# modal-labs/modal-client

Hardware: AMD Instinct MI355X
Metric: map_items_per_sec (higher is better)
Workload: dtype bf16; 1 GPU; model=Function.map fan-out (BASELINE config 3), global_batch=12500, seq_len=0, parallelism=map1, dynamic_batching=64, chunk_items=256, workers=8

## Files before the change

### csrc/core.cpp

```cpp

#include <pybind11/pybind11.h>
#include <pybind11/stl.h>

#include "lane.h"
#include "ring.h"

#include <algorithm>
#include <atomic>
#include <functional>
#include <thread>
#include <cerrno>
#include <cstdint>
#include <cstring>
#include <fcntl.h>
#include <stdexcept>
#include <string>
#include <sys/mman.h>
#include <sys/stat.h>
#include <unistd.h>
#include <vector>

namespace py = pybind11;

namespace {

using modal_amd::BellFile;
using modal_amd::Ring;
using modal_amd::RingHub;

constexpr uint64_t kGilReleaseBytes = 64 * 1024;

bool ring_push(Ring& ring, py::buffer buf) {
  py::buffer_info info = buf.request();
  const uint8_t* src = static_cast<const uint8_t*>(info.ptr);
  const uint64_t n = (uint64_t)info.size * (uint64_t)info.itemsize;
  uint8_t* dst = ring.reserve(n);
  if (!dst) return false;
  if (n >= kGilReleaseBytes) {
    py::gil_scoped_release release;
    std::memcpy(dst, src, n);
  } else {
    std::memcpy(dst, src, n);
  }
  ring.commit();
  return true;
}

py::list ring_pop_all(Ring& ring, size_t max_frames) {
  py::list out;
  ring.pop(
      [&](const uint8_t* ptr, size_t len) {
        out.append(py::bytes(reinterpret_cast<const char*>(ptr), len));
      },
      max_frames);
  return out;
}

py::list hub_drain(RingHub& hub) {
  py::list out;
  hub.drain([&](int slot, const uint8_t* ptr, size_t len) {
    out.append(py::make_tuple(slot, py::bytes(reinterpret_cast<const char*>(ptr), len)));
  });
  return out;
}

using modal_amd::Assignment;
using modal_amd::ChunkDone;
using modal_amd::ChunkLane;
using modal_amd::FrameKind;

py::str sv_str(std::string_view s) { return py::str(s.data(), s.size()); }

py::tuple done_tuple(const ChunkDone& d) {
  py::object cis = py::none();
  if (!d.cis_nil) {
    py::list items;
    for (int64_t v : d.cis) items.append(py::int_(v));
    cis = std::move(items);
// ... 367 lines not shown
    ::close(cg_fd);
    cg_fd = -1;
    throw std::runtime_error("clone3(CLONE_INTO_CGROUP) unavailable: " +
                             std::string(strerror(errno)));
  }
  if (pid < 0) {
    if (cg_fd >= 0) ::close(cg_fd);
    throw std::runtime_error("clone3: " + std::string(strerror(errno)));
  }
  if (pid == 0) {
    ::setsid();
    if (stdin_fd >= 0) ::dup2(stdin_fd, 0);
    if (stdout_fd >= 0) ::dup2(stdout_fd, 1);
    if (stderr_fd >= 0) ::dup2(stderr_fd, 2);
    for (int fd = 3; fd < 1024; ++fd) ::close(fd);
    if (!cwd.empty() && ::chdir(cwd.c_str()) != 0) _exit(126);
    if (rlimit_as_mib > 0) {
      struct rlimit rl;
      rl.rlim_cur = rl.rlim_max = (rlim_t)rlimit_as_mib << 20;
      ::setrlimit(RLIMIT_AS, &rl);
    }
    ::execve(cargv[0], cargv.data(), cenv.data());
    _exit(127);
  }
  if (cg_fd >= 0) ::close(cg_fd);
  return (int64_t)pid;
}


PYBIND11_MODULE(_core, m) {
  m.doc() = "modal_amd native core: shm ring transport + batch framing";
  py::class_<BellFile, std::shared_ptr<BellFile>>(m, "BellFile")
      .def(py::init<const std::string&, bool>(), py::arg("path"), py::arg("create") = false);
  py::class_<Ring, std::shared_ptr<Ring>>(m, "ShmRing")
      .def(py::init<const std::string&, uint64_t, bool>(), py::arg("path"),
           py::arg("capacity") = (uint64_t)64 << 20, py::arg("create") = false)
      .def("push", &ring_push)
      .def("pop_all", &ring_pop_all, py::arg("max_frames") = 0)
      .def("pending_bytes", &Ring::pending_bytes)
      .def("capacity", &Ring::capacity)
      .def("too_large", &Ring::too_large)
      .def("bell_wakes", &Ring::bell_wakes)
      .def("set_shared_bell", &Ring::set_shared_bell);
  py::class_<RingHub>(m, "RingHub")
      .def(py::init<const std::string&, int>(), py::arg("bell_path") = "",
           py::arg("timeout_ms") = 20)
      .def("add_ring", &RingHub::add_ring)
      .def("remove_ring", &RingHub::remove_ring)
      .def("fd", &RingHub::fd)
      .def("drain", &hub_drain)
      .def("close", &RingHub::close)
      .def("stats", [](RingHub& hub) {
        py::dict d;
        d["notifies"] = hub.notifies();
        d["waits"] = hub.waits();
        d["drains"] = hub.drains();
        d["producer_wakes"] = hub.producer_wakes();
        d["rings"] = hub.ring_count();
        return d;
      });
  py::class_<ChunkLane>(m, "ChunkLane")
      .def(py::init<>())
      .def("add_worker", &ChunkLane::add_worker)
      .def("remove_worker", &ChunkLane::remove_worker)
      .def("set_eligible", &ChunkLane::set_eligible)
      .def("set_cap", &ChunkLane::set_cap, py::arg("fn_slot"), py::arg("items"),
           py::arg("min_chunks") = 1)
// ... 30 lines not shown
```

### csrc/lane_stress.cpp

```cpp

#include <poll.h>

#include <atomic>
#include <cstdio>
#include <cstdlib>
#include <map>
#include <string>
#include <thread>
#include <vector>

#include "lane.h"
#include "ring.h"

using namespace modal_amd;

namespace {

constexpr int kWorkers = 2;
constexpr int kChunks = 20000;
constexpr uint64_t kRingBytes = 64 * 1024;
constexpr uint64_t kCount = 64;
constexpr uint64_t kCapItems = 128;
constexpr uint32_t kMinChunks = 2;

#define CHECK(cond)                                                      \
  do {                                                                   \
    if (!(cond)) {                                                       \
      std::fprintf(stderr, "CHECK failed: %s (line %d)\n", #cond, __LINE__); \
      std::abort();                                                      \
    }                                                                    \
  } while (0)

void put_str(std::string& out, const std::string& s) {
  if (s.size() < 32) {
    out.push_back((char)(0xa0 | s.size()));
  } else {
    out.push_back((char)0xd9);
    out.push_back((char)s.size());
  }
  out += s;
}

std::string encode_done(const std::string& token, uint64_t count, const std::string& data) {
  std::string out;
  out.push_back((char)0x88);
  put_str(out, "t");
  put_str(out, "chunk_done");
  put_str(out, "token");
  put_str(out, token);
  put_str(out, "call_id");
  put_str(out, "fc-stress");
  put_str(out, "chunk_id");
  put_str(out, token.substr(2));
  put_str(out, "function_id");
  put_str(out, "fu-stress");
  put_str(out, "count");
  out.push_back((char)count);
  put_str(out, "data");
  out.push_back((char)0xc5);
  out.push_back((char)(data.size() >> 8));
  out.push_back((char)(data.size() & 0xff));
  out += data;
  put_str(out, "cis");
  out.push_back((char)0xc0);
  return out;
}

std::string make_frame(int seq) {
  std::string head = std::to_string(seq) + ":";
  size_t len = 1024 + (size_t)((seq * 2654435761u) % 3072);
  std::string out = head;
  out.resize(len, (char)('a' + seq % 26));
  return out;
}

bool wait_fd(int fd, int timeout_ms) {
  struct pollfd pfd = {fd, POLLIN, 0};
  return ::poll(&pfd, 1, timeout_ms) > 0;
}

}

int main() {
  char dir_template[] = "/tmp/lane-stress-XXXXXX";
  CHECK(::mkdtemp(dir_template) != nullptr);
  std::string dir = dir_template;

  std::vector<std::shared_ptr<Ring>> to_worker_tx, to_worker_rx, from_worker_tx, from_worker_rx;
  for (int i = 0; i < kWorkers; i++) {
    std::string in = dir + "/in." + std::to_string(i), outp = dir + "/out." + std::to_string(i);
    to_worker_tx.push_back(std::make_shared<Ring>(in, kRingBytes, true));
    to_worker_rx.push_back(std::make_shared<Ring>(in, 0, false));
    from_worker_tx.push_back(std::make_shared<Ring>(outp, kRingBytes, true));
    from_worker_rx.push_back(std::make_shared<Ring>(outp, 0, false));
  }

  std::atomic<bool> stop{false};
  std::atomic<int> answered{0};

  std::thread worker([&] {
    RingHub hub(dir + "/worker.bell", 20);
    for (int i = 0; i < kWorkers; i++) hub.add_ring(i, to_worker_rx[i]);
    auto sched_bell = std::make_shared<BellFile>(dir + "/sched.bell", true);
    for (int i = 0; i < kWorkers; i++) from_worker_tx[i]->set_shared_bell(sched_bell);
    std::vector<int> last_seq(kWorkers, -1);
    std::vector<std::pair<int, std::string>> replies;
    while (!stop.load()) {
      wait_fd(hub.fd(), 50);
      replies.clear();
      hub.drain([&](int slot, const uint8_t* ptr, size_t len) {
        std::string body(reinterpret_cast<const char*>(ptr), len);
        int seq = std::atoi(body.c_str());
        CHECK(body == make_frame(seq));
// ... 42 lines not shown
        submitted++;
        if (slot >= 0) assigned(token, slot);
      }
      wait_fd(hub.fd(), 50);
      assignments.clear();
      std::vector<std::pair<int, std::string>> done_now;
      lane.drain(
          hub,
          [&](int slot, const ChunkDone& done) {
            CHECK(done.count == (int64_t)kCount && done.cis_nil);
            CHECK(done.data.size() == (size_t)(std::atoi(done.token.data() + 2) % 700));
            done_now.emplace_back(slot, std::string(done.token));
          },
          [&](int, const uint8_t*, size_t) { CHECK(false && "no raw frames expected"); },
          &assignments);
      for (auto& d : done_now) {
        auto it = where.find(d.second);
        CHECK(it != where.end() && it->second == d.first);
        where.erase(it);
        held[d.first] -= kCount;
        completed++;
      }
      for (auto& a : assignments) assigned(a.token, a.worker_slot);
    }
    CHECK(where.empty() && lane.queued(0) == 0);
    CHECK(lane.pushed() == (uint64_t)kChunks);
    std::printf("lane_stress ok: %d chunks, hub notifies=%llu waits=%llu producer_wakes=%llu\n",
                completed, (unsigned long long)hub.notifies(), (unsigned long long)hub.waits(),
                (unsigned long long)hub.producer_wakes());
    stop.store(true);
    worker.join();
  }
  CHECK(answered.load() == kChunks);
  std::string cmd = "rm -rf " + dir;
  return std::system(cmd.c_str()) == 0 ? 0 : 1;
}
```

### csrc/ring.h

```cpp

#pragma once

#include <atomic>
#include <cerrno>
#include <climits>
#include <cstdint>
#include <cstring>
#include <ctime>
#include <fcntl.h>
#include <linux/futex.h>
#include <memory>
#include <csignal>
#include <pthread.h>
#include <mutex>
#include <stdexcept>
#include <string>
#include <sys/eventfd.h>
#include <sys/mman.h>
#include <sys/stat.h>
#include <sys/syscall.h>
#include <thread>
#include <unistd.h>
#include <utility>
#include <vector>
// ... 92 lines not shown
      ::close(fd_);
      throw std::runtime_error("ShmRing: mmap failed");
    }
    base_ = static_cast<uint8_t*>(mem);
    header_ = reinterpret_cast<RingHeader*>(base_);
    data_ = base_ + sizeof(RingHeader);
    total_ = total;
    if (create) {
      header_->head.store(0, std::memory_order_relaxed);
      header_->tail.store(0, std::memory_order_relaxed);
      header_->capacity = capacity;
      header_->bell.seq.store(0, std::memory_order_relaxed);
      header_->bell.waiting.store(0, std::memory_order_relaxed);
      header_->bell.wakes.store(0, std::memory_order_relaxed);
      header_->magic = kMagic;
    } else if (header_->magic != kMagic || header_->capacity != capacity) {
      ::munmap(base_, total_);
      ::close(fd_);
      throw std::runtime_error("ShmRing: magic mismatch");
    }
    capacity_ = capacity;
  }

  ~Ring() {
    if (base_) ::munmap(base_, total_);
    if (fd_ >= 0) ::close(fd_);
  }

  Ring(const Ring&) = delete;
  Ring& operator=(const Ring&) = delete;

  bool too_large(uint64_t n) const { return n + 8 > capacity_ || n >= kSkip; }

  uint8_t* reserve(uint64_t n) {
    if (too_large(n)) throw std::runtime_error("frame larger than ring");
    uint64_t head = header_->head.load(std::memory_order_relaxed);
    uint64_t tail = header_->tail.load(std::memory_order_acquire);
    uint64_t pos = head % capacity_;
    uint64_t to_end = capacity_ - pos;
    uint64_t need = 4 + n;
    uint64_t skip = to_end < need ? to_end : 0;
    if (head + skip + need - tail > capacity_) return nullptr;
    if (skip) {
      if (to_end >= 4) {
        uint32_t sentinel = kSkip;
        std::memcpy(data_ + pos, &sentinel, 4);
      }
      pos = 0;
    }
    uint32_t len32 = (uint32_t)n;
    std::memcpy(data_ + pos, &len32, 4);
    pending_commit_ = head + skip + need;
    return data_ + pos + 4;
  }

  void commit() {
    header_->head.store(pending_commit_, std::memory_order_release);
    bell_ring(header_->bell);
    if (shared_bell_) bell_ring(*shared_bell_->bell());
  }

  bool push(const uint8_t* src, uint64_t n) {
    uint8_t* dst = reserve(n);
    if (!dst) return false;
    std::memcpy(dst, src, n);
    commit();
    return true;
  }

  template <typename F>
  size_t pop(F&& cb, size_t max_frames = 0) {
    uint64_t tail = header_->tail.load(std::memory_order_relaxed);
    uint64_t head = header_->head.load(std::memory_order_acquire);
    if (tail == head) return 0;
    size_t count = 0;
    while (tail < head) {
      uint64_t pos = tail % capacity_;
      uint64_t to_end = capacity_ - pos;
      if (to_end < 4) {
        tail += to_end;
        continue;
      }
      uint32_t len32;
      std::memcpy(&len32, data_ + pos, 4);
      if (len32 == kSkip) {
        tail += to_end;
        continue;
      }
      if ((uint64_t)len32 + 4 > to_end || tail + 4 + len32 > head) break;
      cb(static_cast<const uint8_t*>(data_ + pos + 4), (size_t)len32);
      tail += 4 + len32;
      if (max_frames && ++count >= max_frames) break;
    }
    header_->tail.store(tail, std::memory_order_release);
    return count;
  }

  bool has_pending() const {
    return header_->head.load(std::memory_order_acquire) !=
           header_->tail.load(std::memory_order_acquire);
  }

  uint64_t pending_bytes() const {
    return header_->head.load(std::memory_order_acquire) -
           header_->tail.load(std::memory_order_acquire);
  }

  uint64_t capacity() const { return capacity_; }
  Bell* bell() const { return &header_->bell; }
  uint32_t bell_wakes() const { return header_->bell.wakes.load(std::memory_order_relaxed); }

  void set_shared_bell(std::shared_ptr<BellFile> bell) { shared_bell_ = std::move(bell); }

 private:
  int fd_ = -1;
  uint8_t* base_ = nullptr;
  uint8_t* data_ = nullptr;
  RingHeader* header_ = nullptr;
  uint64_t capacity_ = 0;
  uint64_t total_ = 0;
  uint64_t pending_commit_ = 0;
  std::shared_ptr<BellFile> shared_bell_;
};

class RingHub {
 public:
  explicit RingHub(const std::string& bell_path = "", int timeout_ms = 20)
      : timeout_ms_(timeout_ms < 1 ? 1 : timeout_ms) {
    if (!bell_path.empty()) {
      bell_file_ = std::make_shared<BellFile>(bell_path, true);
      bell_ = bell_file_->bell();
    }
    efd_ = ::eventfd(0, EFD_NONBLOCK | EFD_CLOEXEC);
    if (efd_ < 0) throw std::runtime_error("RingHub: eventfd failed");
    thread_ = std::thread([this] { run(); });
  }

  ~RingHub() { close(); }
  RingHub(const RingHub&) = delete;
  RingHub& operator=(const RingHub&) = delete;

  void add_ring(int slot, std::shared_ptr<Ring> ring) {
    std::lock_guard<std::mutex> lock(mu_);
    for (auto& entry : rings_) {
      if (entry.first == slot) {
        entry.second = std::move(ring);
        return;
      }
    }
    if (!bell_) {
      bell_owner_ = ring;
      bell_ = ring->bell();
    }
    rings_.emplace_back(slot, std::move(ring));
  }
// ... 118 lines not shown
```

### modal_amd/runtime/worker.py

```python

from __future__ import annotations

import asyncio
import contextvars
import inspect
import os
import sys
import time
import traceback
from concurrent.futures import ThreadPoolExecutor
from typing import Any, Optional

from .._serialization import (
    DataFormat,
    GeneratorDone,
    deserialize,
    deserialize_payload,
    serialize,
    serialize_data_format,
    set_client_context,
)
from ..scheduler.blobs import INLINE_LIMIT, BlobStore
from ..scheduler.calls import (
    GENERIC_STATUS_FAILURE,
# ... 23 lines not shown
    try:
        return (
            cuda is not None
            and os.environ.get("MODAL_AMD_SLOT_STREAMS", "0") not in ("0", "false")
            and cuda.is_initialized()
        )
    except AttributeError:
        return False


def _invoke_on_slot_stream(fn: Any, args: tuple, kwargs: dict) -> Any:
    torch = sys.modules.get("torch")
    cuda = getattr(torch, "cuda", None) if torch is not None else None
    try:
        if (
            cuda is None
            or os.environ.get("MODAL_AMD_SLOT_STREAMS", "0") in ("0", "false")
            or not cuda.is_initialized()
        ):
            return fn(*args, **kwargs)
    except AttributeError:
        return fn(*args, **kwargs)
    stream = getattr(_slot_tls, "stream", None)
    if stream is None:
        stream = torch.cuda.Stream()
        _slot_tls.stream = stream
    with torch.cuda.stream(stream):
        result = fn(*args, **kwargs)
    ev = torch.cuda.Event()
    ev.record(stream)
    torch.cuda.default_stream().wait_event(ev)
    return result

RUNTIME: Optional["WorkerRuntime"] = None


class WorkerRPCTarget:

    def __init__(self, runtime: "WorkerRuntime"):
        self._runtime = runtime

    async def tensor_pull(self, token: str) -> Optional[bytes]:
        tensor = self._runtime.tensor_table.get(token)
        if tensor is None:
            return None
        import pickle as _pickle

        loop = asyncio.get_running_loop()
        return await loop.run_in_executor(
            None, lambda: _pickle.dumps(tensor.detach().cpu(), 4)
        )

    async def ping(self) -> str:
        return self._runtime.task_id

    async def app_stop(self, app_id: str) -> bool:
        await self._runtime._app_teardown(app_id)
        return True

    async def gpu_snapshot(self) -> dict:
        rt = self._runtime
        async with rt.snapshot_lock:
            if rt.mem_snapshot is not None:
                return {"state": rt.mem_snapshot.state.value}
            from .gpu_snapshot import GPUMemorySnapshot

            snap = GPUMemorySnapshot()
            await asyncio.get_running_loop().run_in_executor(None, snap.checkpoint)
            rt.mem_snapshot = snap
            return {"state": snap.state.value}

    async def exec_command(self, cmd: list, timeout: float = 60.0) -> dict:
        proc = await asyncio.create_subprocess_exec(
            *cmd,
            stdout=asyncio.subprocess.PIPE,
            stderr=asyncio.subprocess.STDOUT,
            env=dict(os.environ),
        )
        try:
            out, _ = await asyncio.wait_for(proc.communicate(), timeout)
        except asyncio.TimeoutError:
            proc.kill()
            return {"returncode": -1, "output": "(timed out)"}
        return {"returncode": proc.returncode, "output": out[-65536:].decode(errors="replace")}

    async def gpu_restore(self) -> dict:
        rt = self._runtime
# ... 15 lines not shown
        if float_codec not in (False, True, "auto"):
            raise InvalidError(f'float_codec is False, True or "auto", got {float_codec!r}')
        return await asyncio.get_running_loop().run_in_executor(
            None, capture_manifest, self._runtime.blob_store, float_codec
        )


class FunctionRuntime:

    def __init__(self, runtime: "WorkerRuntime", msg: dict):
        self.runtime = runtime
        self.function_id = msg["function_id"]
        self.app_id = msg.get("app_id", "")
        self.name = msg.get("name", "")
        self.is_generator = bool(msg.get("is_generator"))
        self.timeout = msg.get("timeout")
        self.max_concurrent = max(int(msg.get("max_concurrent_inputs") or 1), 1)
        self.batch_max_size = int(msg.get("batch_max_size") or 0)
        self.batch_linger_ms = int(msg.get("batch_linger_ms") or 0)
        self.version = msg.get("version", 1)
        self.definition_blob = msg["definition"]
        self.definition_kind = msg.get("definition_kind", "serialized")
        self.env = msg.get("env") or {}
        self.volumes = msg.get("volumes") or {}
        self.python_paths = msg.get("python_paths") or []
        self.web_config = msg.get("web_config")
        self._web_runtime: Any = None
        self.sem = asyncio.Semaphore(self.max_concurrent)
        self._callable: Any = None
        self._service: Any = None
        self._loaded = False
        self._load_error: Optional[BaseException] = None
        self._enter_done = False
        self._batch: list[tuple[dict, tuple, dict]] = []
        self._batch_flush_handle: Optional[asyncio.TimerHandle] = None

    def load(self) -> Any:
        if self._loaded:
            if self._load_error is not None:
                raise self._load_error
            return self._callable
        try:
            if self.env:
                os.environ.update(self.env)
            for p in self.python_paths:
                if p not in sys.path:
                    sys.path.insert(0, p)
            if self.volumes:
                from .volumes import mount_volumes

                mount_volumes(self.volumes, self.runtime)
            obj = deserialize(self.definition_blob)
            if isinstance(obj, dict) and obj.get("kind") == "cls_service":
                self._service = _ClsService(obj)
                self._callable = None
            else:
                self._callable = obj
            self._loaded = True
            return self._callable
        except BaseException as exc:
            self._load_error = exc
            self._loaded = True
            raise

    def get_callable(self, method_name: str) -> Any:
        fn = self.load()
# ... 88 lines not shown
        self.gpu_index = (
            int(os.environ["MODAL_AMD_GPU_INDEX"]) if "MODAL_AMD_GPU_INDEX" in os.environ else None
        )
        self.socket_path = os.environ["MODAL_AMD_WORKER_SOCKET"]
        self.external = os.environ.get("MODAL_AMD_EXTERNAL_WORKER") == "1"
        self.conn: Optional[Connection] = None
        self.task_id: str = ""
        self.functions: dict[str, FunctionRuntime] = {}
        self.mem_snapshot: Any = None
        self.snapshot_lock = asyncio.Lock()
        self._sync_threads: dict[str, set] = {}
        self._sync_threads_lock = _threading.Lock()
        self.executor = ThreadPoolExecutor(
            max_workers=int(os.environ.get("MODAL_AMD_WORKER_THREADS", "16")),
            thread_name_prefix="modal-amd-input",
        )
        run_dir = os.path.dirname(self.socket_path)
        self.blob_store = BlobStore(os.path.join(run_dir, "blobs"))
        from .devicemesh import DeviceMesh, TensorTable

        self.mesh = DeviceMesh()
        self.tensor_table = TensorTable()
        self._chunk_cache: dict[str, dict] = {}
        self._chunk_order: list[str] = []
        self._outbox: list[dict] = []
        self._outbox_flush_scheduled = False
        self._running: dict[str, asyncio.Task] = {}
        self._abandoned: set[str] = set()
        self._shutdown = asyncio.Event()
        self._hello_ack = asyncio.Event()
        self._log_buffer: list[tuple[int, str]] = []
        self._log_flush_scheduled = False
        self.loop: Optional[asyncio.AbstractEventLoop] = None

    async def run(self) -> None:
        global RUNTIME
        RUNTIME = self
        self.loop = asyncio.get_running_loop()
        if os.environ.get("MODAL_AMD_RESTORE_STATE_PATH"):
            from .gpu_snapshot import wait_and_restore_from_state_file

            await asyncio.get_running_loop().run_in_executor(
                None, wait_and_restore_from_state_file
            )
        deadline = time.time() + (60.0 if self.external else 0.0)
        while True:
            try:
                reader, writer = await asyncio.open_unix_connection(self.socket_path)
                break
            except (FileNotFoundError, ConnectionRefusedError):
                if time.time() >= deadline:
                    return
                await asyncio.sleep(0.05)
        self.conn = Connection(reader, writer, self._handle, rpc_target=WorkerRPCTarget(self))
        self.conn.start()
        from ..scheduler.core import read_auth_token

        await self.conn.send(
            {
                "t": "hello",
                "role": "worker",
                "worker_id": self.worker_id,
                "gpu_index": self.gpu_index,
                "external": self.external,
                "pid": os.getpid(),
                "auth": read_auth_token(self.socket_path),
# ... 34 lines not shown
            return None
        try:
            free, total = torch.cuda.mem_get_info()
            return {
                "hbm_total": total,
                "hbm_free": free,
                "hbm_reserved": torch.cuda.memory_reserved(),
            }
        except Exception:
            return None

    async def _heartbeat_loop(self) -> None:
        while True:
            await asyncio.sleep(HEARTBEAT_INTERVAL)
            try:
                msg: dict = {"t": "hb"}
                stats = self._gpu_stats()
                if stats:
                    msg["gpu"] = stats
                await self.conn.send(msg)
            except Exception:
                return

    def _handle_sync(self, msg: dict) -> bool:
        if msg.get("t") != "inputs_chunk":
            return False
        frt = self.functions.get(msg["function_id"])
        if frt is None:
            return False
        self._start_chunk(frt, msg)
        return True

    def _start_chunk(self, frt: "FunctionRuntime", msg: dict) -> None:
        task = asyncio.get_running_loop().create_task(self._run_chunk(frt, msg))
        self._running[msg["token"]] = task
        task.add_done_callback(lambda _t, tok=msg["token"]: self._running.pop(tok, None))

    async def _handle(self, msg: dict) -> None:
        kind = msg.get("t")
        if kind == "hello_ack":
            self.task_id = msg.get("task_id", "")
            os.environ["MODAL_AMD_TASK_ID"] = self.task_id
            if msg.get("ring_in"):
                attached = self.conn.attach_rings(
                    msg.get("ring_out"), msg.get("ring_in"), create=False
                )
                if attached and msg.get("lane_bell"):
                    self.conn.sync_handler = self._handle_sync
                    attached = self.conn.enable_lane(shared_bell=msg["lane_bell"], own_hub=True)
                if msg.get("lane_bell") and not attached:
                    sys.__stderr__.write(
                        f"worker {self.worker_id}: cannot attach the native lane, closing\n"
                    )
                    self._shutdown.set()
                    return
            self._hello_ack.set()
        elif kind == "def":
            frt = FunctionRuntime(self, msg)
            self.functions[frt.function_id] = frt
        elif kind == "inputs":
            for cid, data in (msg.get("chunks") or {}).items():
                self._chunk_cache[cid] = {"raw": data, "decoded": None}
                self._chunk_order.append(cid)
                while len(self._chunk_order) > 512:
                    old = self._chunk_order.pop(0)
                    self._chunk_cache.pop(old, None)
            frt = self.functions.get(msg["function_id"])
# ... 255 lines not shown
                vid, ro, _sub = mount_spec(spec)
                if not ro:
                    volume_ids.add(vid)
            if frt._service is not None:
                await asyncio.get_running_loop().run_in_executor(
                    self.executor, frt._service.exit
                )
        if volume_ids:
            await asyncio.get_running_loop().run_in_executor(None, os.sync)
            for volume_id in volume_ids:
                try:
                    await self.conn.call("volume_commit", {"volume_id": volume_id}, timeout=10)
                except Exception:
                    pass

    def _setup_cluster(self, cluster: dict) -> None:
        from ..experimental import ClusterInfo, _set_cluster_info

        rank, size = cluster["rank"], cluster["size"]
        os.environ["RANK"] = str(rank)
        os.environ["WORLD_SIZE"] = str(size)
        os.environ["LOCAL_RANK"] = "0"
        os.environ["MASTER_ADDR"] = "127.0.0.1"
        os.environ["MASTER_PORT"] = str(cluster["master_port"])
        _set_cluster_info(
            ClusterInfo(
                rank=rank,
                cluster_id=cluster["cluster_id"],
                container_ips=["127.0.0.1"] * size,
                fabric_ids=[0] * size,
            )
        )

    async def _run_chunk(self, frt: FunctionRuntime, msg: dict) -> None:
        count = msg["count"]
        token = msg["token"]
        call_id = msg["call_id"]
        self._chunk_cache[msg["chunk_id"]] = {"raw": msg.get("payload"), "decoded": None}
        self._chunk_order.append(msg["chunk_id"])
        while len(self._chunk_order) > 512:
            old = self._chunk_order.pop(0)
            self._chunk_cache.pop(old, None)
        loop = asyncio.get_running_loop()

        values: dict[int, Any] = {}
        errors: dict[int, tuple] = {}

        def run_range(start: int, end: int) -> None:
            try:
                fn = frt.get_callable(msg.get("method", ""))
                pairs, kw_common = self._chunk_pairs(msg["chunk_id"])
            except BaseException as exc:
                data = self._serialize_exception(exc)
                err = "".join(traceback.format_exception_only(type(exc), exc)).strip()
                for ci in range(start, end):
                    errors[ci] = (data, err)
                return
            prefix = f"in-{call_id[3:]}-"
            plain_call = not _slot_streams_enabled()
            tok_c = _current_function_call_id.set(call_id)
            tok_a = _app_id_var.set(frt.app_id)
            self._register_sync_thread(msg["token"])
            try:
                for ci in range(start, end):
                    tok_i = _current_input_id.set(prefix + str(ci))
                    try:
                        if kw_common is None:
                            args, kwargs = pairs[ci]
                        else:
                            args, kwargs = pairs[ci], kw_common
                        if plain_call:
                            values[ci] = fn(*args, **kwargs)
                        else:
                            values[ci] = _invoke_on_slot_stream(fn, args, kwargs)
                    except InputCancellation:
                        raise
                    except BaseException as exc:
                        errors[ci] = (
                            self._serialize_exception(exc),
                            "".join(traceback.format_exception_only(type(exc), exc)).strip(),
                        )
                    finally:
                        _current_input_id.reset(tok_i)
            finally:
                self._unregister_sync_thread(msg["token"])
                _current_function_call_id.reset(tok_c)
                _app_id_var.reset(tok_a)

        from .execution_context import _current_function_call_id, _current_input_id

        try:
            fn0 = await loop.run_in_executor(self.executor, frt.load)
            if frt._service is not None:
                fn0 = frt.get_callable(msg.get("method", ""))
        except BaseException as exc:
            data = self._serialize_exception(exc)
            err = "".join(traceback.format_exception_only(type(exc), exc)).strip()
            for ci in range(count):
                errors[ci] = (data, err)
            fn0 = None

        app_tok = _app_id_var.set(frt.app_id)
        try:
            if fn0 is not None and frt.batch_max_size > 1:
                is_async = inspect.iscoroutinefunction(fn0)

                def _transpose(pairs: Any, kw_common: Any, idxs: range) -> tuple:
                    rows = [
                        (pairs[ci], kw_common) if kw_common is not None else pairs[ci]
                        for ci in idxs
                    ]
                    if kw_common is not None:
                        n_args = len(rows[0][0]) if rows else 0
                        arglists = [[row[0][i] for row in rows] for i in range(n_args)]
                        kwlists = {k: [v] * len(rows) for k, v in kw_common.items()}
                    else:
                        n_args = max((len(a) for a, _ in rows), default=0)
                        arglists = [
                            [a[i] if i < len(a) else None for a, _ in rows]
                            for i in range(n_args)
                        ]
                        keys: set = set()
                        for _, kw in rows:
                            keys.update(kw)
                        kwlists = {k: [kw.get(k) for _, kw in rows] for k in keys}
                    return tuple(arglists), kwlists

                def _store(idxs: range, results: Any) -> None:
                    if not isinstance(results, (list, tuple)) or len(results) != len(idxs):
                        raise ValueError(
                            f"Batched function {frt.name} must return a list of "
                            f"{len(idxs)} results, got {type(results).__name__}"
                        )
                    for ci, r in zip(idxs, results):
                        values[ci] = r

                try:
                    pairs, kw_common = await loop.run_in_executor(
                        self.executor, self._chunk_pairs, msg["chunk_id"]
                    )
                    bsz = frt.batch_max_size
                    async with frt.sem:
                        for start in range(0, count, bsz):
                            idxs = range(start, min(start + bsz, count))
                            try:
                                arglists, kwlists = _transpose(pairs, kw_common, idxs)
                                if is_async:
                                    results = await self._execute(frt, fn0, arglists, kwlists)
                                else:

                                    def _call_batch(
                                        arglists: tuple = arglists, kwlists: dict = kwlists
                                    ) -> Any:
                                        tok_c = _current_function_call_id.set(call_id)
                                        tok_a2 = _app_id_var.set(frt.app_id)
                                        try:
                                            return fn0(*arglists, **kwlists)
                                        finally:
                                            _current_function_call_id.reset(tok_c)
                                            _app_id_var.reset(tok_a2)

                                    results = await loop.run_in_executor(
                                        self.executor, _call_batch
                                    )
                                _store(idxs, results)
                            except (asyncio.CancelledError, InputCancellation):
                                raise
                            except BaseException as exc:
                                data = self._serialize_exception(exc)
                                err = "".join(
                                    traceback.format_exception_only(type(exc), exc)
                                ).strip()
                                for ci in idxs:
                                    errors[ci] = (data, err)
                except (asyncio.CancelledError, InputCancellation):
                    raise
                except BaseException as exc:
                    data = self._serialize_exception(exc)
                    err = "".join(traceback.format_exception_only(type(exc), exc)).strip()
                    for ci in range(count):
                        errors.setdefault(ci, (data, err))
            elif fn0 is not None and (
                inspect.iscoroutinefunction(fn0) or inspect.isasyncgenfunction(fn0)
            ):
                item = {"chunk": msg["chunk_id"], "ci": 0}
                for ci in range(count):
                    item["ci"] = ci
                    try:
                        args, kwargs = await loop.run_in_executor(
                            self.executor, self._resolve_item_args, dict(item)
                        )
                        values[ci] = await self._execute(frt, fn0, args, kwargs)
                    except BaseException as exc:
                        errors[ci] = (
                            self._serialize_exception(exc),
                            "".join(traceback.format_exception_only(type(exc), exc)).strip(),
                        )
            elif fn0 is not None:
                if count <= frt.max_concurrent:
                    n_ranges = count
                else:
                    n_ranges = min(frt.max_concurrent, max(1, count // 16))
                size = (count + n_ranges - 1) // n_ranges

                async def run_one(start: int, end: int) -> None:
                    async with frt.sem:
                        await loop.run_in_executor(self.executor, run_range, start, end)

                await asyncio.gather(
                    *(run_one(s, min(s + size, count)) for s in range(0, count, size))
                )
        except (asyncio.CancelledError, InputCancellation):
            return
        finally:
            _app_id_var.reset(app_tok)

        reply: dict[str, Any] = {
            "t": "chunk_done",
            "token": token,
            "call_id": call_id,
            "chunk_id": msg["chunk_id"],
            "function_id": frt.function_id,
            "count": count,
        }
        if errors:
            reply["exceptions"] = {str(ci): [d, r] for ci, (d, r) in errors.items()}
        if values:
            ordered_cis = sorted(values)
            from ._serialize_chunk import serialize_value_chunk

            def pack() -> tuple:
                return serialize_value_chunk([values[ci] for ci in ordered_cis])

            data, per_item = await loop.run_in_executor(self.executor, pack)
            if data is not None:
                reply["data"] = data
                reply["cis"] = None if len(ordered_cis) == count else ordered_cis
            else:
                reply["items"] = {str(ci): b for ci, b in zip(ordered_cis, per_item)}
        try:
            await self.conn.send(reply)
        except Exception:
            pass

    async def _run_frame_fast(self, frt: FunctionRuntime, items: list[dict]) -> None:
        loop = asyncio.get_running_loop()
        from .execution_context import _current_function_call_id, _current_input_id

        def run_all() -> Any:
            results: list[dict] = []
            try:
                fn = frt.get_callable(items[0].get("method", ""))
            except BaseException as exc:
                err = "".join(traceback.format_exception_only(type(exc), exc)).strip()
                data = self._serialize_exception(exc)
                return [
                    self._make_output(
                        item["token"], frt.function_id, GENERIC_STATUS_FAILURE, data,
                        DataFormat.PICKLE, err,
                    )
                    for item in items
                ]
            if inspect.iscoroutinefunction(fn) or inspect.isasyncgenfunction(fn) or inspect.isgeneratorfunction(fn):
                return None
            values: list = []
            value_tokens: list[str] = []
            for item in items:
                if item["token"] in self._abandoned:
                    self._abandoned.discard(item["token"])
                    continue
                call_id = item["token"].rsplit(":", 2)[0]
                tok_i = _current_input_id.set(item.get("input_id"))
                tok_c = _current_function_call_id.set(call_id)
                try:
                    args, kwargs = self._resolve_item_args(item)
                    values.append(fn(*args, **kwargs))
# ... 51 lines not shown
                        "tokens": value_tokens,
                        "data": chunk_data,
                    }
                )
            except Exception:
                return
            if self._outbox and not self._outbox_flush_scheduled:
                await self._flush_outbox()
            return
        self._outbox.extend(ret)
        if not self._outbox_flush_scheduled:
            await self._flush_outbox()

    def _register_sync_thread(self, token: str) -> None:
        if not token:
            return
        with self._sync_threads_lock:
            self._sync_threads.setdefault(token, set()).add(_threading.get_ident())

    def _unregister_sync_thread(self, token: str) -> None:
        if not token:
            return
        with self._sync_threads_lock:
            idents = self._sync_threads.get(token)
            if idents is not None:
                idents.discard(_threading.get_ident())
                if not idents:
                    self._sync_threads.pop(token, None)

    def _inject_cancel(self, token: str) -> None:
        import ctypes

        with self._sync_threads_lock:
            idents = list(self._sync_threads.get(token, ()))
        for ident in idents:
            ctypes.pythonapi.PyThreadState_SetAsyncExc(
                ctypes.c_ulong(ident), ctypes.py_object(InputCancellation)
            )

    async def _execute(
        self, frt: FunctionRuntime, fn: Any, args: tuple, kwargs: dict, token: str = ""
    ) -> Any:
        from ..utils.tracing import enabled as trace_enabled, trace_range

        if inspect.iscoroutinefunction(fn):
            coro = fn(*args, **kwargs)
            if frt.timeout:
                return await asyncio.wait_for(coro, frt.timeout)
            return await coro
        ctx = contextvars.copy_context()

        def invoke() -> Any:
            self._register_sync_thread(token)
            try:
                if trace_enabled():
                    with trace_range(f"modal_amd::{frt.name}"):
                        return ctx.run(_invoke_on_slot_stream, fn, args, kwargs)
                return ctx.run(_invoke_on_slot_stream, fn, args, kwargs)
            finally:
                self._unregister_sync_thread(token)

        fut = asyncio.get_running_loop().run_in_executor(self.executor, invoke)
        if frt.timeout:
            return await asyncio.wait_for(fut, frt.timeout)
        return await fut

    async def _run_generator(self, frt: FunctionRuntime, fn: Any, token: str, args: tuple, kwargs: dict) -> None:
        index = 0
        if inspect.isasyncgenfunction(fn):
            agen = fn(*args, **kwargs)
            async for value in agen:
# ... 213 lines not shown
```

### modal_amd/scheduler/transport.py

```python

from __future__ import annotations

import asyncio
import os
import itertools
import struct
from collections import deque
from typing import Any, Awaitable, Callable, Optional

import msgpack

_LEN = struct.Struct("<I")

MAX_FRAME = 1 << 31

RING_MIN_FRAME = int(os.environ.get("MODAL_AMD_RING_MIN", 32 * 1024))
RING_CAPACITY = 64 << 20

try:
    from .. import _core
except ImportError:
    _core = None


# ... 13 lines not shown

async def read_frame(reader: asyncio.StreamReader) -> Optional[dict]:
    try:
        header = await reader.readexactly(4)
    except (asyncio.IncompleteReadError, ConnectionResetError):
        return None
    (length,) = _LEN.unpack(header)
    if length > MAX_FRAME:
        raise ValueError(f"Frame too large: {length}")
    try:
        body = await reader.readexactly(length)
    except (asyncio.IncompleteReadError, ConnectionResetError):
        return None
    return msgpack.unpackb(body, raw=False, strict_map_key=False)


class Connection:

    def __init__(
        self,
        reader: asyncio.StreamReader,
        writer: asyncio.StreamWriter,
        handler: Callable[[dict], Awaitable[None]],
        rpc_target: Optional[Any] = None,
    ):
        self.reader = reader
        self.writer = writer
        self.handler = handler
        self.rpc_target = rpc_target
        self._rpc_seq = itertools.count(1)
        self._pending: dict[int, asyncio.Future] = {}
        self._send_lock = asyncio.Lock()
        self._closed = asyncio.Event()
        self._reader_task: Optional[asyncio.Task] = None
        self._loop: Optional[asyncio.AbstractEventLoop] = None
        self.ring_out: Any = None
        self.ring_in: Any = None
        self.ring_frames_sent = 0
        self.ring_frames_received = 0
        self._lane = False
        self._own_hub: Any = None
        self.sync_handler: Optional[Callable[[dict], bool]] = None
        self._inbox: deque = deque()
        self._lane_waiting = 0
        self._inbox_task: Optional[asyncio.Task] = None

    def attach_rings(self, out_path: Optional[str], in_path: Optional[str], create: bool) -> bool:
        if _core is None or not out_path or not in_path:
            return False
        try:
            self.ring_out = _core.ShmRing(out_path, RING_CAPACITY, create)
            self.ring_in = _core.ShmRing(in_path, RING_CAPACITY, create)
            return True
        except Exception:
            self.ring_out = None
            self.ring_in = None
            return False

    def enable_lane(self, shared_bell: Optional[str] = None, own_hub: bool = False) -> bool:
        if _core is None or self.ring_out is None or self.ring_in is None:
            return False
        try:
            if shared_bell:
                self.ring_out.set_shared_bell(_core.BellFile(shared_bell, False))
            if own_hub:
                hub = _core.RingHub("", 20)
# ... 36 lines not shown

    async def _run_inbox(self) -> None:
        try:
            while self._inbox:
                msg = self._inbox.popleft()
                try:
                    await self._dispatch(msg)
                except asyncio.CancelledError:
                    raise
                except Exception:
                    pass
        finally:
            self._inbox_task = None
            if self._inbox and not self._closed.is_set():
                self._inbox_task = asyncio.get_running_loop().create_task(self._run_inbox())

    async def _send_lane(self, body: bytes) -> None:
        if self._closed.is_set():
            raise ConnectionError("connection closed")
        ring = self.ring_out
        if self._lane_waiting == 0 and ring.push(body):
            self.ring_frames_sent += 1
            return
        self._lane_waiting += 1
        try:
            async with self._send_lock:
                while not ring.push(body):
                    if self._closed.is_set():
                        raise ConnectionError("connection closed")
                    await asyncio.sleep(0.001)
                self.ring_frames_sent += 1
        finally:
            self._lane_waiting -= 1

    def start(self) -> None:
        self._loop = asyncio.get_running_loop()
        self._reader_task = self._loop.create_task(self._read_loop())

    @property
    def closed(self) -> bool:
        return self._closed.is_set()

    async def wait_closed(self) -> None:
        await self._closed.wait()

    async def send(self, msg: dict, via_socket: bool = False) -> None:
        body = msgpack.packb(msg, use_bin_type=True)
        if self._lane and not via_socket:
            await self._send_lane(body)
            return
        if self.ring_out is not None and len(body) >= RING_MIN_FRAME and not via_socket:
            pushed = self.ring_out.push(body)
            if pushed:
                self.ring_frames_sent += 1
                async with self._send_lock:
                    self.writer.write(pack({"t": "rb"}))
                    await self.writer.drain()
                return
        data = _LEN.pack(len(body)) + body
        async with self._send_lock:
            self.writer.write(data)
            await self.writer.drain()

    async def call(self, method: str, params: Any = None, timeout: Optional[float] = None) -> Any:
        running = asyncio.get_running_loop()
        if self._loop is not None and running is not self._loop:
# ... 44 lines not shown
            raise
        except BaseException as exc:
            await self.send(
                {"t": "rpc_e", "i": rpc_id, "e": f"{type(exc).__name__}: {exc}", "c": type(exc).__name__}
            )

    async def _read_loop(self) -> None:
        try:
            while True:
                msg = await read_frame(self.reader)
                if msg is None:
                    break
                if msg.get("t") == "rb":
                    if self.ring_in is not None:
                        for body in self.ring_in.pop_all():
                            self.ring_frames_received += 1
                            await self._dispatch(
                                msgpack.unpackb(body, raw=False, strict_map_key=False)
                            )
                    continue
                await self._dispatch(msg)
        except asyncio.CancelledError:
            pass
        except Exception:
            pass
        finally:
            if self._lane and self.ring_in is not None:
                try:
                    for body in self.ring_in.pop_all():
                        self.on_ring_frame(body)
                except Exception:
                    pass
            self._drop_own_hub()
            self._closed.set()
            for fut in self._pending.values():
                if not fut.done():
                    fut.set_exception(ConnectionError("connection closed"))
            try:
                self.writer.close()
            except Exception:
                pass

    async def close(self) -> None:
        if self._reader_task is not None:
            self._reader_task.cancel()
        self._drop_own_hub()
        try:
            self.writer.close()
            await self.writer.wait_closed()
        except Exception:
            pass
        self._closed.set()


class RemoteRPCError(Exception):
    def __init__(self, message: str, code: Optional[str] = None):
        super().__init__(message)
        self.code = code
```

Measured before the change: 1.604 million items/s.

## Run sync batched chunks entirely in executor thread and push replies from thread

For batched sync functions, the whole chunk (decode, batched calls, reply serialization, msgpack) now runs as one executor job, and the reply is pushed straight into the shared-memory ring from the worker thread. This avoids per-batch event-loop round trips and executor hops. To make that safe, Ring::push gains a producer mutex so several threads can produce concurrently. Stats counters are added, and a multi-producer stress test covers the ring. The costs are extra lock traffic and more complex cancellation and fallback paths.

```diff
diff --git a/csrc/core.cpp b/csrc/core.cpp
--- a/csrc/core.cpp
+++ b/csrc/core.cpp
@@ -34,16 +34,12 @@
   py::buffer_info info = buf.request();
   const uint8_t* src = static_cast<const uint8_t*>(info.ptr);
   const uint64_t n = (uint64_t)info.size * (uint64_t)info.itemsize;
-  uint8_t* dst = ring.reserve(n);
-  if (!dst) return false;
+  if (ring.too_large(n)) throw std::runtime_error("frame larger than ring");
   if (n >= kGilReleaseBytes) {
     py::gil_scoped_release release;
-    std::memcpy(dst, src, n);
-  } else {
-    std::memcpy(dst, src, n);
-  }
-  ring.commit();
-  return true;
+    return ring.push(src, n);
+  }
+  return ring.push(src, n);
 }
 
 py::list ring_pop_all(Ring& ring, size_t max_frames) {
@@ -477,7 +473,9 @@
   m.doc() = "modal_amd native core: shm ring transport + batch framing";
   py::class_<BellFile, std::shared_ptr<BellFile>>(m, "BellFile")
       .def(py::init<const std::string&, bool>(), py::arg("path"), py::arg("create") = false);
-  py::class_<Ring, std::shared_ptr<Ring>>(m, "ShmRing")
+  py::class_<Ring, std::shared_ptr<Ring>> ring_cls(m, "ShmRing");
+  m.attr("Ring") = ring_cls;
+  ring_cls
       .def(py::init<const std::string&, uint64_t, bool>(), py::arg("path"),
            py::arg("capacity") = (uint64_t)64 << 20, py::arg("create") = false)
       .def("push", &ring_push)
diff --git a/csrc/lane_stress.cpp b/csrc/lane_stress.cpp
--- a/csrc/lane_stress.cpp
+++ b/csrc/lane_stress.cpp
@@ -22,6 +22,7 @@
 constexpr uint64_t kCount = 64;
 constexpr uint64_t kCapItems = 128;
 constexpr uint32_t kMinChunks = 2;
+constexpr uint64_t kCountMax = (uint64_t)1 << 40;
 
 #define CHECK(cond)                                                      \
   do {                                                                   \
@@ -79,6 +80,79 @@
   return ::poll(&pfd, 1, timeout_ms) > 0;
 }
 
+
+constexpr int kProducers = 3;
+constexpr int kFramesOf[kProducers] = {8000, 4000, 8000};
+
+std::string make_tagged(int id, int seq) {
+  static const size_t base[kProducers] = {64, 8 * 1024, 1024};
+  static const size_t span[kProducers] = {256, 12 * 1024, 3072};
+  std::string out = "P" + std::to_string(id) + ":" + std::to_string(seq) + ":";
+  size_t len = base[id] + (size_t)((seq * 2654435761u) % span[id]);
+  out.resize(len, (char)('A' + (seq + id) % 26));
+  return out;
+}
+
+void run_multi_producer(const std::string& dir) {
+  std::string path = dir + "/mp.ring";
+  auto tx = std::make_shared<Ring>(path, kRingBytes, true);
+  auto rx = std::make_shared<Ring>(path, 0, false);
+  RingHub hub(dir + "/mp.bell", 20);
+  hub.add_ring(0, rx);
+  tx->set_shared_bell(std::make_shared<BellFile>(dir + "/mp.bell", true));
+
+  auto push_direct = [&](int id) {
+    for (int seq = 0; seq < kFramesOf[id]; seq++) {
+      std::string frame = make_tagged(id, seq);
+      const auto* ptr = reinterpret_cast<const uint8_t*>(frame.data());
+      while (!tx->push(ptr, frame.size())) std::this_thread::yield();
+    }
+  };
+  auto push_through_lane = [&](int id) {
+    ChunkLane lane;
+    lane.add_worker(0, tx);
+    lane.set_eligible(0, 0, true);
+    lane.set_cap(0, kCountMax, 1);
+    std::vector<Assignment> refilled;
+    for (int seq = 0; seq < kFramesOf[id]; seq++) {
+      std::string frame = make_tagged(id, seq);
+      std::string token = "m:" + std::to_string(seq);
+      int slot = lane.submit(0, token, 1, reinterpret_cast<const uint8_t*>(frame.data()),
+                             frame.size(), false);
+      while (slot < 0 && lane.queued(0)) {
+        std::this_thread::yield();
+        lane.kick(0, &refilled);
+      }
+      CHECK(lane.complete(0, token, &refilled));
+    }
+    CHECK(lane.pushed() == (uint64_t)kFramesOf[id] && lane.queued(0) == 0);
+  };
+
+  std::thread small(push_direct, 0), large(push_direct, 1), laned(push_through_lane, 2);
+  int next[kProducers] = {0, 0, 0};
+  int total = 0, want = kFramesOf[0] + kFramesOf[1] + kFramesOf[2];
+  while (total < want) {
+    wait_fd(hub.fd(), 50);
+    hub.drain([&](int, const uint8_t* ptr, size_t len) {
+      std::string body(reinterpret_cast<const char*>(ptr), len);
+      CHECK(len > 4 && body[0] == 'P' && body[2] == ':');
+      int id = body[1] - '0';
+      CHECK(id >= 0 && id < kProducers);
+      int seq = std::atoi(body.c_str() + 3);
+      CHECK(seq == next[id]);
+      CHECK(body == make_tagged(id, seq));
+      next[id]++;
+      total++;
+    });
+  }
+  small.join();
+  large.join();
+  laned.join();
+  for (int id = 0; id < kProducers; id++) CHECK(next[id] == kFramesOf[id]);
+  CHECK(!rx->has_pending());
+  std::printf("lane_stress multi-producer: %d frames from %d threads\n", total, kProducers);
+}
+
 }
 
 int main() {
@@ -187,6 +261,8 @@
     worker.join();
   }
   CHECK(answered.load() == kChunks);
+  run_multi_producer(dir);
+  std::printf("lane_stress ok\n");
   std::string cmd = "rm -rf " + dir;
   return std::system(cmd.c_str()) == 0 ? 0 : 1;
 }
diff --git a/csrc/ring.h b/csrc/ring.h
--- a/csrc/ring.h
+++ b/csrc/ring.h
@@ -148,6 +148,60 @@
 
   bool too_large(uint64_t n) const { return n + 8 > capacity_ || n >= kSkip; }
 
+  bool push(const uint8_t* src, uint64_t n) {
+    std::lock_guard<std::mutex> lock(producer_mu_);
+    uint8_t* dst = reserve(n);
+    if (!dst) return false;
+    std::memcpy(dst, src, n);
+    commit();
+    return true;
+  }
+
+  template <typename F>
+  size_t pop(F&& cb, size_t max_frames = 0) {
+    uint64_t tail = header_->tail.load(std::memory_order_relaxed);
+    uint64_t head = header_->head.load(std::memory_order_acquire);
+    if (tail == head) return 0;
+    size_t count = 0;
+    while (tail < head) {
+      uint64_t pos = tail % capacity_;
+      uint64_t to_end = capacity_ - pos;
+      if (to_end < 4) {
+        tail += to_end;
+        continue;
+      }
+      uint32_t len32;
+      std::memcpy(&len32, data_ + pos, 4);
+      if (len32 == kSkip) {
+        tail += to_end;
+        continue;
+      }
+      if ((uint64_t)len32 + 4 > to_end || tail + 4 + len32 > head) break;
+      cb(static_cast<const uint8_t*>(data_ + pos + 4), (size_t)len32);
+      tail += 4 + len32;
+      if (max_frames && ++count >= max_frames) break;
+    }
+    header_->tail.store(tail, std::memory_order_release);
+    return count;
+  }
+
+  bool has_pending() const {
+    return header_->head.load(std::memory_order_acquire) !=
+           header_->tail.load(std::memory_order_acquire);
+  }
+
+  uint64_t pending_bytes() const {
+    return header_->head.load(std::memory_order_acquire) -
+           header_->tail.load(std::memory_order_acquire);
+  }
+
+  uint64_t capacity() const { return capacity_; }
+  Bell* bell() const { return &header_->bell; }
+  uint32_t bell_wakes() const { return header_->bell.wakes.load(std::memory_order_relaxed); }
+
+  void set_shared_bell(std::shared_ptr<BellFile> bell) { shared_bell_ = std::move(bell); }
+
+ private:
   uint8_t* reserve(uint64_t n) {
     if (too_large(n)) throw std::runtime_error("frame larger than ring");
     uint64_t head = header_->head.load(std::memory_order_relaxed);
@@ -176,59 +230,6 @@
     if (shared_bell_) bell_ring(*shared_bell_->bell());
   }
 
-  bool push(const uint8_t* src, uint64_t n) {
-    uint8_t* dst = reserve(n);
-    if (!dst) return false;
-    std::memcpy(dst, src, n);
-    commit();
-    return true;
-  }
-
-  template <typename F>
-  size_t pop(F&& cb, size_t max_frames = 0) {
-    uint64_t tail = header_->tail.load(std::memory_order_relaxed);
-    uint64_t head = header_->head.load(std::memory_order_acquire);
-    if (tail == head) return 0;
-    size_t count = 0;
-    while (tail < head) {
-      uint64_t pos = tail % capacity_;
-      uint64_t to_end = capacity_ - pos;
-      if (to_end < 4) {
-        tail += to_end;
-        continue;
-      }
-      uint32_t len32;
-      std::memcpy(&len32, data_ + pos, 4);
-      if (len32 == kSkip) {
-        tail += to_end;
-        continue;
-      }
-      if ((uint64_t)len32 + 4 > to_end || tail + 4 + len32 > head) break;
-      cb(static_cast<const uint8_t*>(data_ + pos + 4), (size_t)len32);
-      tail += 4 + len32;
-      if (max_frames && ++count >= max_frames) break;
-    }
-    header_->tail.store(tail, std::memory_order_release);
-    return count;
-  }
-
-  bool has_pending() const {
-    return header_->head.load(std::memory_order_acquire) !=
-           header_->tail.load(std::memory_order_acquire);
-  }
-
-  uint64_t pending_bytes() const {
-    return header_->head.load(std::memory_order_acquire) -
-           header_->tail.load(std::memory_order_acquire);
-  }
-
-  uint64_t capacity() const { return capacity_; }
-  Bell* bell() const { return &header_->bell; }
-  uint32_t bell_wakes() const { return header_->bell.wakes.load(std::memory_order_relaxed); }
-
-  void set_shared_bell(std::shared_ptr<BellFile> bell) { shared_bell_ = std::move(bell); }
-
- private:
   int fd_ = -1;
   uint8_t* base_ = nullptr;
   uint8_t* data_ = nullptr;
@@ -237,6 +238,7 @@
   uint64_t total_ = 0;
   uint64_t pending_commit_ = 0;
   std::shared_ptr<BellFile> shared_bell_;
+  std::mutex producer_mu_;
 };
 
 class RingHub {
diff --git a/modal_amd/runtime/worker.py b/modal_amd/runtime/worker.py
--- a/modal_amd/runtime/worker.py
+++ b/modal_amd/runtime/worker.py
@@ -79,6 +79,40 @@
     torch.cuda.default_stream().wait_event(ev)
     return result
 
+def _transpose_batch(pairs: Any, kw_common: Any, idxs: range) -> tuple:
+    rows = [
+        (pairs[ci], kw_common) if kw_common is not None else pairs[ci]
+        for ci in idxs
+    ]
+    if kw_common is not None:
+        n_args = len(rows[0][0]) if rows else 0
+        arglists = [[row[0][i] for row in rows] for i in range(n_args)]
+        kwlists = {k: [v] * len(rows) for k, v in kw_common.items()}
+    else:
+        n_args = max((len(a) for a, _ in rows), default=0)
+        arglists = [
+            [a[i] if i < len(a) else None for a, _ in rows]
+            for i in range(n_args)
+        ]
+        keys: set = set()
+        for _, kw in rows:
+            keys.update(kw)
+        kwlists = {k: [kw.get(k) for _, kw in rows] for k in keys}
+    return tuple(arglists), kwlists
+
+
+def _store_batch(name: str, values: dict, idxs: range, results: Any) -> None:
+    if not isinstance(results, (list, tuple)) or len(results) != len(idxs):
+        raise ValueError(
+            f"Batched function {name} must return a list of "
+            f"{len(idxs)} results, got {type(results).__name__}"
+        )
+    for ci, r in zip(idxs, results):
+        values[ci] = r
+
+
+_NOT_SYNC = object()
+
 RUNTIME: Optional["WorkerRuntime"] = None
 
 
@@ -100,6 +134,9 @@
 
     async def ping(self) -> str:
         return self._runtime.task_id
+
+    async def chunk_stats(self) -> dict:
+        return self._runtime.chunk_stats()
 
     async def app_stop(self, app_id: str) -> bool:
         await self._runtime._app_teardown(app_id)
@@ -181,6 +218,7 @@
         self._loaded = False
         self._load_error: Optional[BaseException] = None
         self._enter_done = False
+        self._chunk_job_ok: dict[str, bool] = {}
         self._batch: list[tuple[dict, tuple, dict]] = []
         self._batch_flush_handle: Optional[asyncio.TimerHandle] = None
 
@@ -335,6 +373,23 @@
         self._log_buffer: list[tuple[int, str]] = []
         self._log_flush_scheduled = False
         self.loop: Optional[asyncio.AbstractEventLoop] = None
+        self._chunk_stats = {
+            "chunks": 0,
+            "executor_jobs": 0,
+            "thread_replies": 0,
+            "loop_replies": 0,
+            "chunk_wall_ns": 0,
+        }
+        self._chunk_stats_lock = _threading.Lock()
+
+    def chunk_stats(self) -> dict:
+        with self._chunk_stats_lock:
+            return dict(self._chunk_stats)
+
+    def _chunk_stat_add(self, **deltas: int) -> None:
+        with self._chunk_stats_lock:
+            for key, delta in deltas.items():
+                self._chunk_stats[key] += delta
 
     async def run(self) -> None:
         global RUNTIME
@@ -435,7 +490,10 @@
         return True
 
     def _start_chunk(self, frt: "FunctionRuntime", msg: dict) -> None:
-        task = asyncio.get_running_loop().create_task(self._run_chunk(frt, msg))
+        self._chunk_stat_add(chunks=1)
+        task = asyncio.get_running_loop().create_task(
+            self._run_chunk(frt, msg, time.perf_counter_ns())
+        )
         self._running[msg["token"]] = task
         task.add_done_callback(lambda _t, tok=msg["token"]: self._running.pop(tok, None))
 
@@ -757,7 +815,7 @@
             )
         )
 
-    async def _run_chunk(self, frt: FunctionRuntime, msg: dict) -> None:
+    async def _run_chunk(self, frt: FunctionRuntime, msg: dict, t_start: int = 0) -> None:
         count = msg["count"]
         token = msg["token"]
         call_id = msg["call_id"]
@@ -767,6 +825,10 @@
             old = self._chunk_order.pop(0)
             self._chunk_cache.pop(old, None)
         loop = asyncio.get_running_loop()
+
+        if frt.batch_max_size > 1 and frt._chunk_job_ok.get(msg.get("method", ""), True):
+            if await self._run_chunk_job(frt, msg, t_start):
+                return
 
         values: dict[int, Any] = {}
         errors: dict[int, tuple] = {}
@@ -830,36 +892,6 @@
             if fn0 is not None and frt.batch_max_size > 1:
                 is_async = inspect.iscoroutinefunction(fn0)
 
-                def _transpose(pairs: Any, kw_common: Any, idxs: range) -> tuple:
-                    rows = [
-                        (pairs[ci], kw_common) if kw_common is not None else pairs[ci]
-                        for ci in idxs
-                    ]
-                    if kw_common is not None:
-                        n_args = len(rows[0][0]) if rows else 0
-                        arglists = [[row[0][i] for row in rows] for i in range(n_args)]
-                        kwlists = {k: [v] * len(rows) for k, v in kw_common.items()}
-                    else:
-                        n_args = max((len(a) for a, _ in rows), default=0)
-                        arglists = [
-                            [a[i] if i < len(a) else None for a, _ in rows]
-                            for i in range(n_args)
-                        ]
-                        keys: set = set()
-                        for _, kw in rows:
-                            keys.update(kw)
-                        kwlists = {k: [kw.get(k) for _, kw in rows] for k in keys}
-                    return tuple(arglists), kwlists
-
-                def _store(idxs: range, results: Any) -> None:
-                    if not isinstance(results, (list, tuple)) or len(results) != len(idxs):
-                        raise ValueError(
-                            f"Batched function {frt.name} must return a list of "
-                            f"{len(idxs)} results, got {type(results).__name__}"
-                        )
-                    for ci, r in zip(idxs, results):
-                        values[ci] = r
-
                 try:
                     pairs, kw_common = await loop.run_in_executor(
                         self.executor, self._chunk_pairs, msg["chunk_id"]
@@ -869,7 +901,7 @@
                         for start in range(0, count, bsz):
                             idxs = range(start, min(start + bsz, count))
                             try:
-                                arglists, kwlists = _transpose(pairs, kw_common, idxs)
+                                arglists, kwlists = _transpose_batch(pairs, kw_common, idxs)
                                 if is_async:
                                     results = await self._execute(frt, fn0, arglists, kwlists)
                                 else:
@@ -888,7 +920,7 @@
                                     results = await loop.run_in_executor(
                                         self.executor, _call_batch
                                     )
-                                _store(idxs, results)
+                                _store_batch(frt.name, values, idxs, results)
                             except (asyncio.CancelledError, InputCancellation):
                                 raise
                             except BaseException as exc:
@@ -940,10 +972,20 @@
         finally:
             _app_id_var.reset(app_tok)
 
+        if values:
+            reply = await loop.run_in_executor(
+                self.executor, self._chunk_reply, frt, msg, values, errors
+            )
+        else:
+            reply = self._chunk_reply(frt, msg, values, errors)
+        await self._send_chunk_reply(reply, t_start)
+
+    def _chunk_reply(self, frt: FunctionRuntime, msg: dict, values: dict, errors: dict) -> dict:
+        count = msg["count"]
         reply: dict[str, Any] = {
             "t": "chunk_done",
-            "token": token,
-            "call_id": call_id,
+            "token": msg["token"],
+            "call_id": msg["call_id"],
             "chunk_id": msg["chunk_id"],
             "function_id": frt.function_id,
             "count": count,
@@ -954,19 +996,131 @@
             ordered_cis = sorted(values)
             from ._serialize_chunk import serialize_value_chunk
 
-            def pack() -> tuple:
-                return serialize_value_chunk([values[ci] for ci in ordered_cis])
-
-            data, per_item = await loop.run_in_executor(self.executor, pack)
+            data, per_item = serialize_value_chunk([values[ci] for ci in ordered_cis])
             if data is not None:
                 reply["data"] = data
                 reply["cis"] = None if len(ordered_cis) == count else ordered_cis
             else:
                 reply["items"] = {str(ci): b for ci, b in zip(ordered_cis, per_item)}
+        return reply
+
+    async def _send_chunk_reply(self, reply: dict, t_start: int) -> None:
         try:
             await self.conn.send(reply)
         except Exception:
             pass
+        self._chunk_stat_add(
+            loop_replies=1, chunk_wall_ns=time.perf_counter_ns() - t_start if t_start else 0
+        )
+
+    async def _run_chunk_job(self, frt: FunctionRuntime, msg: dict, t_start: int) -> bool:
+        from .execution_context import _current_function_call_id
+
+        loop = asyncio.get_running_loop()
+        count = msg["count"]
+        token = msg["token"]
+        call_id = msg["call_id"]
+        method = msg.get("method", "")
+        bsz = frt.batch_max_size
+        cancelled = [False]
+
+        def job() -> Any:
+            values: dict[int, Any] = {}
+            errors: dict[int, tuple] = {}
+            tok_c = _current_function_call_id.set(call_id)
+            tok_a = _app_id_var.set(frt.app_id)
+            self._register_sync_thread(token)
+            try:
+                fn = pairs = kw_common = None
+                try:
+                    fn = frt.get_callable(method)
+                    if inspect.iscoroutinefunction(fn):
+                        return _NOT_SYNC
+                    pairs, kw_common = self._chunk_pairs(msg["chunk_id"])
+                except InputCancellation:
+                    raise
+                except BaseException as exc:
+                    data = self._serialize_exception(exc)
+                    err = "".join(traceback.format_exception_only(type(exc), exc)).strip()
+                    for ci in range(count):
+                        errors[ci] = (data, err)
+                self._chunk_stat_add(executor_jobs=1)
+                for start in range(0, count, bsz) if not errors else ():
+                    if cancelled[0]:
+                        raise InputCancellation()
+                    idxs = range(start, min(start + bsz, count))
+                    try:
+                        arglists, kwlists = _transpose_batch(pairs, kw_common, idxs)
+                        _store_batch(frt.name, values, idxs, fn(*arglists, **kwlists))
+                    except InputCancellation:
+                        raise
+                    except BaseException as exc:
+                        data = self._serialize_exception(exc)
+                        err = "".join(traceback.format_exception_only(type(exc), exc)).strip()
+                        for ci in idxs:
+                            errors[ci] = (data, err)
+                reply = self._chunk_reply(frt, msg, values, errors)
+                clean = "data" in reply and "exceptions" not in reply and "items" not in reply
+                if clean and not cancelled[0]:
+                    import msgpack
+
+                    body = msgpack.packb(reply, use_bin_type=True)
+                    self._chunk_stat_add(thread_replies=1)
+                    if self.conn.try_push_from_thread(body):
+                        if t_start:
+                            self._chunk_stat_add(chunk_wall_ns=time.perf_counter_ns() - t_start)
+                        return None
+                    self._chunk_stat_add(thread_replies=-1)
+                return reply
+            finally:
+                try:
+                    _current_function_call_id.reset(tok_c)
+                    _app_id_var.reset(tok_a)
+                finally:
+                    self._unregister_sync_thread(token)
+
+        try:
+            await frt.sem.acquire()
+        except asyncio.CancelledError:
+            return True
+        done: asyncio.Future = loop.create_future()
+
+        def on_loop(cfut: Any) -> None:
+            frt.sem.release()
+            if done.done():
+                return
+            if cfut.cancelled():
+                done.cancel()
+            elif cfut.exception() is not None:
+                done.set_exception(cfut.exception())
+            else:
+                done.set_result(cfut.result())
+
+        def on_job_end(cfut: Any) -> None:
+            try:
+                loop.call_soon_threadsafe(on_loop, cfut)
+            except RuntimeError:
+                pass
+
+        try:
+            cfut = self.executor.submit(job)
+        except BaseException:
+            frt.sem.release()
+            raise
+        cfut.add_done_callback(on_job_end)
+        try:
+            reply = await done
+        except (asyncio.CancelledError, InputCancellation):
+            cancelled[0] = True
+            return True
+        if reply is _NOT_SYNC:
+            frt._chunk_job_ok[method] = False
+            return False
+        if reply is None:
+            self.conn.ring_frames_sent += 1
+            return True
+        await self._send_chunk_reply(reply, t_start)
+        return True
 
     async def _run_frame_fast(self, frt: FunctionRuntime, items: list[dict]) -> None:
         loop = asyncio.get_running_loop()
@@ -1084,11 +1238,10 @@
         import ctypes
 
         with self._sync_threads_lock:
-            idents = list(self._sync_threads.get(token, ()))
-        for ident in idents:
-            ctypes.pythonapi.PyThreadState_SetAsyncExc(
-                ctypes.c_ulong(ident), ctypes.py_object(InputCancellation)
-            )
+            for ident in self._sync_threads.get(token, ()):
+                ctypes.pythonapi.PyThreadState_SetAsyncExc(
+                    ctypes.c_ulong(ident), ctypes.py_object(InputCancellation)
+                )
 
     async def _execute(
         self, frt: FunctionRuntime, fn: Any, args: tuple, kwargs: dict, token: str = ""
diff --git a/modal_amd/scheduler/transport.py b/modal_amd/scheduler/transport.py
--- a/modal_amd/scheduler/transport.py
+++ b/modal_amd/scheduler/transport.py
@@ -69,6 +69,7 @@
         self._pending: dict[int, asyncio.Future] = {}
         self._send_lock = asyncio.Lock()
         self._closed = asyncio.Event()
+        self._closed_flag = False
         self._reader_task: Optional[asyncio.Task] = None
         self._loop: Optional[asyncio.AbstractEventLoop] = None
         self.ring_out: Any = None
@@ -171,6 +172,15 @@
                 self.ring_frames_sent += 1
         finally:
             self._lane_waiting -= 1
+
+    def try_push_from_thread(self, body: bytes) -> bool:
+        ring = self.ring_out
+        if not self._lane or ring is None or self._closed_flag or self._lane_waiting:
+            return False
+        try:
+            return bool(ring.push(body))
+        except Exception:
+            return False
 
     def start(self) -> None:
         self._loop = asyncio.get_running_loop()
@@ -281,6 +291,7 @@
                 except Exception:
                     pass
             self._drop_own_hub()
+            self._closed_flag = True
             self._closed.set()
             for fut in self._pending.values():
                 if not fut.done():
@@ -299,6 +310,7 @@
             await self.writer.wait_closed()
         except Exception:
             pass
+        self._closed_flag = True
         self._closed.set()
 
 
```

New measurement: 1.683 million items/s, median of 5. 4.9% higher.
